# yaramohamadi/Pairwise_Sample_Optimization

Hardware: AMD Instinct MI355X
Metric: PSO train-step imgs/sec (paired 1024² SDXL) at 1/2/4/8 MI355X (higher is better)
Workload: dtype bf16; 1 GPU; C2: SDXL-Turbo PSO train step, LoRA r=32 grads, 2 pairs/GPU/micro-step, gas 2, 2-step sampler (T=1); global_batch=4, seq_len=4096, resolution=1024, parallelism=dp1, launch=eager

## Files before the change

### include/pso_amd.h

```cpp
#ifndef PSO_AMD_H
#define PSO_AMD_H

#include <stddef.h>
#include <stdint.h>

#ifdef __cplusplus
extern "C" {
#endif

#define PSO_ABI_VERSION 1

#define PSO_OK 0
#define PSO_ERR_ARG 1
#define PSO_ERR_HIP 2
#define PSO_ERR_UNSUPPORTED 3

#define PSO_F32 0
#define PSO_BF16 1
#define PSO_F16 2
#define PSO_U8 2

#define PSO_MODE_TURBO 0
#define PSO_MODE_DMD 1
#define PSO_MODE_DMD_F16 2
// ... 85 lines not shown
                    float grad_scale, void* deps, int deps_dtype, const void* ws, size_t ws_bytes, void* stream);

#define PSO_CONV_NORMAL 1
#define PSO_CONV_UP2 2
#define PSO_CONV_T2 3
int pso_conv2d(int mode, int B, const void* src1, int C1, const void* src2, int C2, int H, int W, int Ho, int Wo,
               int ks, int stride, int pad, const void* weight, int Cout, const void* a2, long lda2, int K2,
               const void* b2, long ldb2, float alpha, const void* bias, const void* rowbias, long ld_rowbias,
               const void* resid, long ldr, void* out, long ldo, int out_dtype, int accumulate, void* stream);
size_t pso_conv2d_ws_bytes(int B, int Ho, int Wo, int Cout, int K1, int K2);
int pso_conv2d_ws(int mode, int B, const void* src1, int C1, const void* src2, int C2, int H, int W, int Ho, int Wo,
                  int ks, int stride, int pad, const void* weight, int Cout, const void* a2, long lda2, int K2,
                  const void* b2, long ldb2, float alpha, const void* bias, const void* rowbias, long ld_rowbias,
                  const void* resid, long ldr, void* out, long ldo, int out_dtype, int accumulate, void* ws,
                  size_t ws_bytes, void* stream);

size_t pso_group_norm_ws_bytes(int B, int HW, int C);
int pso_group_norm_fwd(int B, int HW, int C, int G, float eps, const void* x, const void* gamma, const void* beta,
                       int silu, void* y, float* stats, void* ws, size_t ws_bytes, void* stream);
int pso_group_norm_bwd(int B, int HW, int C, int G, const void* x, const void* dy, const float* stats,
                       const void* gamma, const void* beta, int silu, const void* dadd, void* dx, float* dgamma,
                       float* dbeta, int accumulate_dparams, void* ws, size_t ws_bytes, void* stream);

int pso_layer_norm_fwd(int M, int C, float eps, const void* x, long ldx, const void* gamma, const void* beta, void* y,
                       long ldy, float* stats, void* stream);
int pso_layer_norm_bwd(int M, int C, const void* x, long ldx, const void* dy, long lddy, const float* stats,
                       const void* gamma, const void* dadd, long ldadd, void* dx, long lddx, void* stream);

int pso_attention_fwd(int B, int H, int Sq, int Sk, const void* q, long ldq, long sq_b, const void* k, long ldk,
                      long sk_b, const void* v, long ldv, long sv_b, float scale, void* o, long ldo, long so_b,
// ... 124 lines not shown
```

### pairwise_sample_optimization_amd/_lib.py

```python
import ctypes
import os

import torch

_HERE = os.path.dirname(os.path.abspath(__file__))
KNOBS = os.environ.get("PSO_LIB", "") == "knobs"
F16 = os.environ.get("PSO_LIB", "") == "f16"
LIB_PATH = os.environ.get("PSO_LIB_PATH") or os.path.join(
    _HERE, "libpso_amd_knobs.so" if KNOBS else "libpso_amd_f16.so" if F16 else "libpso_amd.so")

PSO_F32 = 0
PSO_BF16 = 1
PSO_F16 = 2
ELEM_DTYPE = torch.float16 if F16 else torch.bfloat16
ELEM_CODE = PSO_F16 if F16 else PSO_BF16
MODE_TURBO = 0
MODE_DMD = 1
MODE_DMD_F16 = 2
MODE_DMD_BF16 = 3
COEF_STRIDE = 8
AMP_WORDS = 16
(AMP_SCALE, AMP_INV_SCALE, AMP_FOUND_INF, AMP_GROWTH_TRACKER, AMP_STEP, AMP_SKIPPED, AMP_NORM, AMP_CLIP_COEF,
 AMP_GRAD_MUL, AMP_BC1, AMP_BC2_SQRT, AMP_C1, AMP_C2) = range(13)
AMP_INT_WORDS = (AMP_FOUND_INF, AMP_GROWTH_TRACKER, AMP_STEP, AMP_SKIPPED)
# ... 49 lines not shown
    "pso_gemm_tn_ws": (ci, [ci, ci, ci, vp, cl, vp, cl, cf, vp, cl, vp, csz, vp]),
    "pso_gemm_tn_rank_batch": (ci, [ci, ci, ci, vp, vp]),
    "pso_gemm_tn_rank_batch_ws_bytes": (csz, [ci, ci, ci, vp]),
    "pso_gemm_tn_rank_batch_ws": (ci, [ci, ci, ci, vp, vp, csz, vp]),
    "pso_gemm_skinny_grouped": (ci, [ci, ci, ci, vp, cl, vp, cl, cf, vp, cl, ci, vp]),
    "pso_gemm_geglu": (ci, [ci, ci, vp, cl, ci, vp, cl, vp, vp, cl, vp, cl, ci, vp]),
    "pso_gemm_geglu_bwd": (ci, [ci, ci, vp, cl, ci, vp, cl, vp, cl, vp, cl, vp]),
    "pso_quant_rows_fp8": (ci, [ci, ci, vp, cl, vp, cl, vp, vp]),
    "pso_gemm_fp8": (ci, [ci, ci, ci, ci, vp, cl, vp, vp, cl, vp, vp, cl, ci, vp, vp, cl, vp, ci, ci, cf, vp, vp, cl,
                          vp, cl, vp, cl, ci, vp]),
    "pso_conv2d": (ci, [ci, ci, vp, ci, vp, ci, ci, ci, ci, ci, ci, ci, ci, vp, ci, vp, cl, ci, vp, cl, cf, vp, vp,
                        cl, vp, cl, vp, cl, ci, ci, vp]),
    "pso_conv2d_ws_bytes": (csz, [ci, ci, ci, ci, ci, ci]),
    "pso_conv2d_ws": (ci, [ci, ci, vp, ci, vp, ci, ci, ci, ci, ci, ci, ci, ci, vp, ci, vp, cl, ci, vp, cl, cf, vp, vp,
                           cl, vp, cl, vp, cl, ci, ci, vp, csz, vp]),
    "pso_group_norm_ws_bytes": (csz, [ci, ci, ci]),
    "pso_group_norm_fwd": (ci, [ci, ci, ci, ci, cf, vp, vp, vp, ci, vp, vp, vp, csz, vp]),
    "pso_group_norm_bwd": (ci, [ci, ci, ci, ci, vp, vp, vp, vp, vp, ci, vp, vp, vp, vp, ci, vp, csz, vp]),
    "pso_layer_norm_fwd": (ci, [ci, ci, cf, vp, cl, vp, vp, vp, cl, vp, vp]),
    "pso_layer_norm_bwd": (ci, [ci, ci, vp, cl, vp, cl, vp, vp, vp, cl, vp, cl, vp]),
    "pso_attention_fwd": (ci, [ci, ci, ci, ci, vp, cl, cl, vp, cl, cl, vp, cl, cl, cf, vp, cl, cl, vp, vp]),
    "pso_attention_bwd_ws_bytes": (csz, [ci, ci, ci, ci]),
    "pso_attention_bwd": (ci, [ci, ci, ci, ci, vp, cl, cl, vp, cl, cl, vp, cl, cl, vp, cl, cl, vp, vp, cl, cl, cf,
                               vp, cl, cl, vp, cl, cl, vp, cl, cl, vp, csz, vp]),
    "pso_geglu_fwd": (ci, [cl, ci, vp, cl, vp, cl, vp]),
    "pso_geglu_bwd": (ci, [cl, ci, vp, cl, vp, cl, vp, cl, vp]),
    "pso_silu": (ci, [cl, vp, vp, vp]),
    "pso_timestep_embedding": (ci, [ci, ci, vp, vp, cl, ci, vp]),
    "pso_transpose": (ci, [ci, ci, ci, vp, cl, vp, cl, vp]),
    "pso_im2col3": (ci, [ci, ci, ci, ci, vp, vp, ci, vp]),
# ... 129 lines not shown
```

### pairwise_sample_optimization_amd/csrc/elementwise.hip

```cpp
#include "common.h"

__device__ __forceinline__ void unpack8e(uint4 v, float* f) {
  const uint32_t w[4] = {v.x, v.y, v.z, v.w};
#pragma unroll
  for (int i = 0; i < 4; ++i) {
    f[2 * i] = bf2f(w[i] & 0xffff);
    f[2 * i + 1] = bf2f(w[i] >> 16);
  }
}
__device__ __forceinline__ uint4 pack8e(const float* f) {
  return make_uint4(pack2bf(f[0], f[1]), pack2bf(f[2], f[3]), pack2bf(f[4], f[5]), pack2bf(f[6], f[7]));
}

static int grid_for(long n, int per_thread = 1) {
  long g = (n / per_thread + 255) / 256;
  if (g > 8192) g = 8192;
  return (int)(g < 1 ? 1 : g);
}

#define GRID_STRIDE(i, n) for (long i = blockIdx.x * (long)blockDim.x + threadIdx.x; i < (n); i += (long)gridDim.x * blockDim.x)


__global__ void geglu_fwd_kernel(long M, int F, const bf16_t* __restrict__ in, long ldi, bf16_t* __restrict__ out,
                                 long ldo) {
// ... 209 lines not shown
    const bf16_t* src = w + co * ldw + (long)tap * Ci + ci;
    if (vec && co < Co && ci + 8 <= Ci) {
      *reinterpret_cast<uint4*>(&tile[r][c]) = *reinterpret_cast<const uint4*>(src);
    } else {
      for (int e = 0; e < 8; ++e) tile[r][c + e] = (co < Co && ci + e < Ci) ? src[e] : (bf16_t)0;
    }
  }
  __syncthreads();
  const int lx = t & 63, ly = t >> 6;
  for (int i = ly; i < 64; i += 4) {
    const int ci = ci0 + i, co = co0 + lx;
    if (ci < Ci && co < Co) wt[((long)ci * ks * ks + tap2) * Co + co] = tile[lx][i];
  }
}

__global__ void concat_kernel(long npix, int C1, const bf16_t* __restrict__ x1, int C2, const bf16_t* __restrict__ x2,
                              bf16_t* __restrict__ out) {
  const int C8 = (C1 + C2) / 8, c18 = C1 / 8;
  GRID_STRIDE(v, npix * C8) {
    const long p = v / C8;
    const int ch = (int)(v - p * C8);
    const uint4 val = ch < c18 ? *reinterpret_cast<const uint4*>(x1 + p * C1 + ch * 8)
                               : *reinterpret_cast<const uint4*>(x2 + p * C2 + (ch - c18) * 8);
    *reinterpret_cast<uint4*>(out + v * 8) = val;
  }
}

__global__ void split_kernel(long npix, int C1, int C2, const bf16_t* __restrict__ in, bf16_t* __restrict__ y1,
                             bf16_t* __restrict__ y2, const bf16_t* __restrict__ add2) {
  const int C8 = (C1 + C2) / 8, c18 = C1 / 8;
// ... 236 lines not shown
  cast_f32_bf16_kernel<<<grid_for(n, 8), 256, 0, (hipStream_t)stream>>>(n, x, scale, (bf16_t*)y);
  return pso_check_launch("pso_cast_f32_bf16");
}

int pso_cast_bf16_f32(long n, const void* x, float* y, void* stream) {
  cast_bf16_f32_kernel<<<grid_for(n, 8), 256, 0, (hipStream_t)stream>>>(n, (const bf16_t*)x, y);
  return pso_check_launch("pso_cast_bf16_f32");
}

int pso_conv_weight_t(int Co, int ks, int Ci, int flip, const void* w, void* wt, void* stream) {
  conv_weight_t_kernel<<<dim3(cdiv(Ci, 64), cdiv(Co, 64), ks * ks), 256, 0, (hipStream_t)stream>>>(
      Co, ks, Ci, flip, (const bf16_t*)w, (bf16_t*)wt);
  return pso_check_launch("pso_conv_weight_t");
}

}
```

### pairwise_sample_optimization_amd/csrc/gemm.hip

```cpp
#include "common.h"

#include <cstdlib>

#define GEMM_THREADS 256
#define BK 64

struct ConvGeom {
  int mode;
  const bf16_t* src2;
  int C1, C2;
  int H, W;
  int Ho, Wo;
  int ks, stride, pad;
};

struct GemmArgs {
  const bf16_t* a1; long lda1; int K1;
  const bf16_t* b1; long ldb1;
  const bf16_t* a2; long lda2; int K2;
  const bf16_t* b2; long ldb2;
  int tail_group_n;
  int tail_m;
  int M, N;
  ConvGeom conv;
// ... 151 lines not shown
  const int nt2 = (g.a2 && m0 < g.tail_m) ? (g.K2 + BK - 1) / BK : 0;
  const int nt_all = nt1 + nt2;
  const int per = (nt_all + gridDim.y - 1) / gridDim.y;
  const int t_beg = blockIdx.y * per;
  const int t_end = min(nt_all, t_beg + per);
  const int nt = t_end > t_beg ? t_end - t_beg : 0;
  const long a2_off = g.tail_group_n > 0 ? (long)(n0 / g.tail_group_n) * g.K2 : 0;

  const int prow = lane >> 3;
  const int pch = lane & 7;
  const bf16_t* zero = reinterpret_cast<const bf16_t*>(g_zero16);
  const long zb = blockIdx.z;
  const bf16_t* const a1 = g.a1 + zb * g.bat_a;
  const bf16_t* const b1 = g.b1 + zb * g.bat_b;
  void* const outp = reinterpret_cast<char*>(g.out) + zb * g.bat_o * (g.out_dtype == PSO_F32 ? 4 : 2);
  const int K1 = g.K1;
  int lcA[T::A_CH], offA[T::A_CH];
  int lcB[T::B_CH], offB[T::B_CH];
  RowCoord rc[T::A_CH];
#pragma unroll
  for (int i = 0; i < T::A_CH; ++i) {
    const int R = pa(i) * 8 + prow;
    const int m = min(m0 + R, g.M - 1);
    lcA[i] = pch ^ (R & 7);
    offA[i] = CONV ? 0 : (int)((long)m * g.lda1) + lcA[i] * 8;
    if (CONV) {
      const int hw = g.conv.Ho * g.conv.Wo;
      rc[i].valid = true;
      rc[i].b = m / hw;
      const int rem = m - rc[i].b * hw;
// ... 21 lines not shown
        const TapInfo ti = tap_info(g, k0);
#pragma unroll
        for (int i = 0; i < T::A_CH; ++i) {
          const int piece = pa(i);
          int iy, ix;
          bool ok;
          if (CONV == PSO_CONV_NORMAL) {
            iy = rc[i].oy * cvS + ti.kh - cvP;
            ix = rc[i].ox * cvS + ti.kw - cvP;
            ok = (unsigned)iy < (unsigned)cvH && (unsigned)ix < (unsigned)cvW;
          } else if (CONV == PSO_CONV_UP2) {
            const int uy = rc[i].oy + ti.kh - cvP, ux = rc[i].ox + ti.kw - cvP;
            ok = (unsigned)uy < (unsigned)(2 * cvH) && (unsigned)ux < (unsigned)(2 * cvW);
            iy = uy >> 1;
            ix = ux >> 1;
          } else {
            const int ty = rc[i].oy + cvP - ti.kh, tx = rc[i].ox + cvP - ti.kw;
            iy = ty >> 1;
            ix = tx >> 1;
            ok = ty >= 0 && tx >= 0 && !(ty & 1) && !(tx & 1) && iy < cvH && ix < cvW;
          }
          const bf16_t* src = ti.src + ((long)((rc[i].b * cvH + iy) * cvW + ix)) * ti.Cs + ti.c0 + lcA[i] * 8;
          __builtin_amdgcn_global_load_lds(static_cast<const void*>(ok ? src : zero), (lds_void*)(la + piece * 8 * BK), 16, 0, 0);
        }
      } else {
#pragma unroll
        for (int i = 0; i < T::A_CH; ++i) {
          const int piece = pa(i);
          const bool ok = full || k0 + lcA[i] * 8 < K1;
          __builtin_amdgcn_global_load_lds(static_cast<const void*>(ok ? a1 + offA[i] + k0 : zero), (lds_void*)(la + piece * 8 * BK), 16, 0, 0);
// ... 308 lines not shown
#pragma unroll
      for (int it = 0; it < ITERS; ++it) {
        const int q = threadIdx.x + it * NT;
        const int ml = q / CC, cl = (q - (q / CC) * CC) * 8;
        const int m = m0 + ml;
        if (q >= BM * CC || m >= g.M) continue;
        uint4 y = *reinterpret_cast<const uint4*>(tl + ml * TP + cl);
        if (g.resid) {
          const uint32_t yw[4] = {y.x, y.y, y.z, y.w}, rw[4] = {rr[it].x, rr[it].y, rr[it].z, rr[it].w};
          uint32_t o[4];
#pragma unroll
          for (int e = 0; e < 4; ++e)
            o[e] = pack2bf(bf2f(yw[e] & 0xffff) + bf2f(rw[e] & 0xffff), bf2f(yw[e] >> 16) + bf2f(rw[e] >> 16));
          y = make_uint4(o[0], o[1], o[2], o[3]);
        }
        *reinterpret_cast<uint4*>(reinterpret_cast<bf16_t*>(outp) + (long)m * g.ldo + n0 + cl) = y;
      }
      return;
    }
  }
  if (!PIPE && epi_fast && nt > 0) {
    epi_prefetch();
    const bool has_add = g.resid || g.rowbias;
#pragma unroll
    for (int i = 0; i < MI; ++i) {
      const int m = m0 + wm * (BM / WM) + i * 16 + fr;
      if (m >= g.M) continue;
#pragma unroll
      for (int j = 0; j < NJ; ++j) {
        const int n = n0 + wn * (BN / WN) + j * 16 + fk * 4;
        float v[4] = {acc[i][j][0] * g.alpha + bf2f(ebias[j].x & 0xffff), acc[i][j][1] * g.alpha + bf2f(ebias[j].x >> 16),
                      acc[i][j][2] * g.alpha + bf2f(ebias[j].y & 0xffff), acc[i][j][3] * g.alpha + bf2f(ebias[j].y >> 16)};
        if (has_add) {
          v[0] += bf2f(eadd[i][j].x & 0xffff); v[1] += bf2f(eadd[i][j].x >> 16);
          v[2] += bf2f(eadd[i][j].y & 0xffff); v[3] += bf2f(eadd[i][j].y >> 16);
        }
        if (g.out_dtype == PSO_ELEM) {
          *reinterpret_cast<uint2*>(reinterpret_cast<bf16_t*>(outp) + (long)m * g.ldo + n) =
              make_uint2(pack2bf(v[0], v[1]), pack2bf(v[2], v[3]));
        } else {
          float4* o = reinterpret_cast<float4*>(reinterpret_cast<float*>(outp) + (long)m * g.ldo + n);
          if (g.accumulate) {
            const float4 old = *o;
            v[0] += old.x; v[1] += old.y; v[2] += old.z; v[3] += old.w;
          }
          *o = make_float4(v[0], v[1], v[2], v[3]);
        }
      }
    }
    return;
  }
#pragma unroll
  for (int i = 0; i < MI; ++i) {
    const int m = m0 + wm * (BM / WM) + i * 16 + fr;
    if (m >= g.M) continue;
#pragma unroll
    for (int j = 0; j < NJ; ++j) {
      const int n = n0 + wn * (BN / WN) + j * 16 + fk * 4;
      if (n >= g.N) continue;
      float v[4] = {acc[i][j][0] * g.alpha, acc[i][j][1] * g.alpha, acc[i][j][2] * g.alpha,
                    acc[i][j][3] * g.alpha};
      if (gridDim.y > 1) {
        float* o = reinterpret_cast<float*>(outp) + (long)m * g.ldo + n;
        for (int r = 0; r < 4 && n + r < g.N; ++r) atomicAdd(o + r, v[r]);
        continue;
      }
      const bool full = g.vec_ok && (n + 4 <= g.N);
      if (full) {
        if (g.bias) {
          const uint2 bv = *reinterpret_cast<const uint2*>(g.bias + n);
          v[0] += bf2f(bv.x & 0xffff); v[1] += bf2f(bv.x >> 16); v[2] += bf2f(bv.y & 0xffff); v[3] += bf2f(bv.y >> 16);
        }
        if (g.rowbias) {
          const uint2 bv = *reinterpret_cast<const uint2*>(g.rowbias + (long)(m / g.rows_per_group) * g.ld_rowbias + n);
          v[0] += bf2f(bv.x & 0xffff); v[1] += bf2f(bv.x >> 16); v[2] += bf2f(bv.y & 0xffff); v[3] += bf2f(bv.y >> 16);
        }
        if (g.resid) {
          const uint2 rv = *reinterpret_cast<const uint2*>(g.resid + (long)m * g.ldr + n);
          v[0] += bf2f(rv.x & 0xffff); v[1] += bf2f(rv.x >> 16); v[2] += bf2f(rv.y & 0xffff); v[3] += bf2f(rv.y >> 16);
        }
        if (g.out_dtype == PSO_ELEM) {
          *reinterpret_cast<uint2*>(reinterpret_cast<bf16_t*>(outp) + (long)m * g.ldo + n) =
              make_uint2(pack2bf(v[0], v[1]), pack2bf(v[2], v[3]));
        } else {
          float4* o = reinterpret_cast<float4*>(reinterpret_cast<float*>(outp) + (long)m * g.ldo + n);
          if (g.accumulate) {
            const float4 old = *o;
            v[0] += old.x; v[1] += old.y; v[2] += old.z; v[3] += old.w;
          }
          *o = make_float4(v[0], v[1], v[2], v[3]);
        }
      } else {
        for (int r = 0; r < 4 && n + r < g.N; ++r) {
          float x = v[r];
          if (g.bias) x += bf2f(g.bias[n + r]);
          if (g.rowbias) x += bf2f(g.rowbias[(long)(m / g.rows_per_group) * g.ld_rowbias + n + r]);
          if (g.resid) x += bf2f(g.resid[(long)m * g.ldr + n + r]);
          if (g.out_dtype == PSO_ELEM) {
            reinterpret_cast<bf16_t*>(outp)[(long)m * g.ldo + n + r] = f2bf(x);
          } else {
            float* o = reinterpret_cast<float*>(outp) + (long)m * g.ldo + n + r;
            *o = g.accumulate ? *o + x : x;
          }
        }
      }
    }
  }
}

template <int BM, int BN, int WM = 2, int WN = 2, int STAGES = 2, bool PIPE = false, int EPI = EPI_NONE>
static int launch(const GemmArgs& g, hipStream_t st, int ksplit = 1) {
  const int nblk = ((g.M + BM - 1) / BM) * ((g.N + BN - 1) / BN);
  dim3 grid(nblk, ksplit, g.batch > 1 ? g.batch : 1);
  const int threads = 64 * WM * WN;
  const size_t shm = (size_t)STAGES * (BM + BN) * BK * sizeof(bf16_t);
  pso_note_kernel("gemm_bf16_kernel<%d, %d, %d, %d, %d, %d, %s, %d>", BM, BN, EPI != EPI_NONE ? 0 : g.conv.mode, WM, WN,
                  STAGES, PIPE ? "true" : "false", EPI);
  static bool attr_done = false;
  if constexpr (EPI != EPI_NONE) {
    if (!attr_done) {
      (void)hipFuncSetAttribute((const void*)gemm_bf16_kernel<BM, BN, 0, WM, WN, STAGES, PIPE, EPI>,
                                hipFuncAttributeMaxDynamicSharedMemorySize, (int)shm);
      attr_done = true;
    }
    gemm_bf16_kernel<BM, BN, 0, WM, WN, STAGES, PIPE, EPI><<<grid, threads, shm, st>>>(g);
    return pso_check_launch("pso_gemm(geglu)");
  }
  if (!attr_done) {
    (void)hipFuncSetAttribute((const void*)gemm_bf16_kernel<BM, BN, 0, WM, WN, STAGES, PIPE, EPI>,
                        hipFuncAttributeMaxDynamicSharedMemorySize, (int)shm);
    (void)hipFuncSetAttribute((const void*)gemm_bf16_kernel<BM, BN, PSO_CONV_NORMAL, WM, WN, STAGES, PIPE, EPI>,
                        hipFuncAttributeMaxDynamicSharedMemorySize, (int)shm);
    (void)hipFuncSetAttribute((const void*)gemm_bf16_kernel<BM, BN, PSO_CONV_UP2, WM, WN, STAGES, PIPE, EPI>,
                        hipFuncAttributeMaxDynamicSharedMemorySize, (int)shm);
    (void)hipFuncSetAttribute((const void*)gemm_bf16_kernel<BM, BN, PSO_CONV_T2, WM, WN, STAGES, PIPE, EPI>,
                        hipFuncAttributeMaxDynamicSharedMemorySize, (int)shm);
    attr_done = true;
  }
  switch (g.conv.mode) {
    case PSO_CONV_NORMAL:
      gemm_bf16_kernel<BM, BN, PSO_CONV_NORMAL, WM, WN, STAGES, PIPE, EPI><<<grid, threads, shm, st>>>(g);
      break;
    case PSO_CONV_UP2: gemm_bf16_kernel<BM, BN, PSO_CONV_UP2, WM, WN, STAGES, PIPE, EPI><<<grid, threads, shm, st>>>(g); break;
    case PSO_CONV_T2: gemm_bf16_kernel<BM, BN, PSO_CONV_T2, WM, WN, STAGES, PIPE, EPI><<<grid, threads, shm, st>>>(g); break;
    default: gemm_bf16_kernel<BM, BN, 0, WM, WN, STAGES, PIPE, EPI><<<grid, threads, shm, st>>>(g);
  }
  return pso_check_launch("pso_gemm");
}

static bool al16(const void* p) { return ((uintptr_t)p & 15) == 0; }
static bool al8(const void* p) { return ((uintptr_t)p & 7) == 0; }

// ... 102 lines not shown
  g.group_m = g_gemm_group > 0 ? g_gemm_group : PSO_GEMM_GROUP_M;
  if (g.tail_group_n > 0 && (g.tail_group_n % 64) != 0) {
    pso_set_error("pso_gemm: tail_group_n must be a multiple of 64");
    return PSO_ERR_ARG;
  }
  g.stage_epi = gv_raw != 41 && g.out_dtype == PSO_ELEM && al16(g.out) && (g.ldo % 8) == 0 &&
                (!g.resid || (al16(g.resid) && (g.ldr % 8) == 0));
  g.vec_ok = (g.ldo % 4) == 0 && (g.out_dtype == PSO_F32 ? al16(g.out) : al8(g.out)) &&
             (!g.resid || ((g.ldr % 4) == 0 && al8(g.resid))) && (!g.bias || al8(g.bias)) &&
             (!g.rowbias || (al8(g.rowbias) && (g.ld_rowbias % 4) == 0));
  const bool bn64_only = g.tail_group_n > 0 && (g.tail_group_n % 128) != 0;
  const bool bn256_ok = g.tail_group_n == 0 || (g.tail_group_n % 256) == 0;
  const long Ktot = (long)g.K1 + (g.a2 ? g.K2 : 0);
  if (g.batch > 1) {
    auto tl = [&](int bm, int bn) { return (long)((g.M + bm - 1) / bm) * ((g.N + bn - 1) / bn) * g.batch; };
    if ((g.N % 160) == 0 && tl(128, 160) >= 256) return launch<128, 160, 2, 2, 2>(g, st);
    if (tl(128, 128) >= 256) return launch<128, 128, 2, 4, 2>(g, st);
    return launch<64, 64>(g, st);
  }
  if (g.ws) {
    const SplitPlan sp = gemm_split_plan(g.M, g.N, g.K1, g.K2, g.a2 != nullptr, true);
    if (sp.ks >= 2) {
      if (sp.bn == 160) launch<128, 160, 2, 2, 2>(g, st, sp.ks);
      else launch<128, 128, 2, 4, 2>(g, st, sp.ks);
      const long n4 = (long)g.M * (g.N / 4);
      gemm_splitk_reduce_kernel<<<(unsigned)((n4 + 255) / 256), 256, 0, st>>>(g, sp.ks);
      return pso_check_launch("pso_gemm_ws");
    }
    g.ws = nullptr;
  }
// ... 678 lines not shown
  g.alpha = alpha; g.rows_per_group = 1;
  g.out = out; g.ldo = ldo; g.out_dtype = out_dtype;
  g.bat_a = stride_a; g.bat_b = stride_b; g.bat_o = stride_o; g.batch = batch;
  return run_gemm(g, (hipStream_t)stream);
}

int pso_conv2d(int mode, int B, const void* src1, int C1, const void* src2, int C2, int H, int W, int Ho, int Wo,
               int ks, int stride, int pad, const void* weight, int Cout, const void* a2, long lda2, int K2,
               const void* b2, long ldb2, float alpha, const void* bias, const void* rowbias, long ld_rowbias,
               const void* resid, long ldr, void* out, long ldo, int out_dtype, int accumulate, void* stream) {
  PSO_ARG_CHECK(mode == PSO_CONV_NORMAL || mode == PSO_CONV_UP2 || mode == PSO_CONV_T2, "pso_conv2d: bad mode");
  PSO_ARG_CHECK(src1 && weight && out, "pso_conv2d: null operand");
  PSO_ARG_CHECK((C1 % 64) == 0 && (C2 % 64) == 0 && (C2 == 0 || src2),
                "pso_conv2d: channel sources must be multiples of 64 (C1=%d C2=%d); use im2col for small C", C1, C2);
  PSO_ARG_CHECK(al16(src1) && (!src2 || al16(src2)) && al16(weight), "pso_conv2d: alignment");
  PSO_ARG_CHECK(ks == 1 || ks == 3, "pso_conv2d: ks must be 1 or 3");
  PSO_ARG_CHECK(mode != PSO_CONV_UP2 || (Ho == 2 * H && Wo == 2 * W && stride == 1), "pso_conv2d: UP2 geometry");
  PSO_ARG_CHECK(!a2 || ((K2 % 8) == 0 && b2 && al16(a2) && al16(b2)), "pso_conv2d: bad second operand");
  PSO_DTYPE_CHECK(out_dtype, "pso_conv2d");
  PSO_ARG_CHECK(!accumulate || out_dtype == PSO_F32, "pso_conv2d: accumulate needs f32 output");
  if (mode == PSO_CONV_NORMAL && ks == 3 && stride == 1 && pad == 1 && Ho == H && Wo == W && C2 == 0 && !a2 &&
      !rowbias && !resid && alpha == 1.f && out_dtype == PSO_ELEM && !accumulate && ldo == Cout && Cout <= 3 &&
      pso_conv3x3_smallc_run(B, H, W, C1, Cout, src1, weight, bias, out, (hipStream_t)stream) == PSO_OK)
    return PSO_OK;
  GemmArgs g{};
  const int Ct = C1 + C2;
  g.a1 = (const bf16_t*)src1; g.lda1 = 0; g.K1 = ks * ks * Ct;
  g.b1 = (const bf16_t*)weight; g.ldb1 = g.K1;
  g.a2 = (const bf16_t*)a2; g.lda2 = lda2; g.K2 = a2 ? K2 : 0;
  g.b2 = (const bf16_t*)b2; g.ldb2 = ldb2;
  g.M = B * Ho * Wo; g.N = Cout;
// ... 13 lines not shown
  if (M <= 0 || M > 0x7fffffffL) return 0;
  const SplitPlan sp = gemm_split_plan((int)M, Cout, K1, K2, K2 > 0, true);
  return sp.ks >= 2 ? (size_t)sp.ks * M * Cout * sizeof(float) : 0;
}

int pso_conv2d_ws(int mode, int B, const void* src1, int C1, const void* src2, int C2, int H, int W, int Ho, int Wo,
                  int ks, int stride, int pad, const void* weight, int Cout, const void* a2, long lda2, int K2,
                  const void* b2, long ldb2, float alpha, const void* bias, const void* rowbias, long ld_rowbias,
                  const void* resid, long ldr, void* out, long ldo, int out_dtype, int accumulate, void* ws,
                  size_t ws_bytes, void* stream) {
  PSO_ARG_CHECK(mode == PSO_CONV_NORMAL || mode == PSO_CONV_UP2 || mode == PSO_CONV_T2, "pso_conv2d_ws: bad mode");
  PSO_ARG_CHECK(src1 && weight && out, "pso_conv2d_ws: null operand");
  PSO_ARG_CHECK((C1 % 64) == 0 && (C2 % 64) == 0 && (C2 == 0 || src2),
                "pso_conv2d_ws: channel sources must be multiples of 64 (C1=%d C2=%d)", C1, C2);
  PSO_ARG_CHECK(al16(src1) && (!src2 || al16(src2)) && al16(weight), "pso_conv2d_ws: alignment");
  PSO_ARG_CHECK(ks == 1 || ks == 3, "pso_conv2d_ws: ks must be 1 or 3");
  PSO_ARG_CHECK(mode != PSO_CONV_UP2 || (Ho == 2 * H && Wo == 2 * W && stride == 1), "pso_conv2d_ws: UP2 geometry");
  PSO_ARG_CHECK(!a2 || ((K2 % 8) == 0 && b2 && al16(a2) && al16(b2)), "pso_conv2d_ws: bad second operand");
  PSO_DTYPE_CHECK(out_dtype, "pso_conv2d_ws");
  PSO_ARG_CHECK(!accumulate || out_dtype == PSO_F32, "pso_conv2d_ws: accumulate needs f32 output");
  GemmArgs g{};
  const int Ct = C1 + C2;
  g.a1 = (const bf16_t*)src1; g.lda1 = 0; g.K1 = ks * ks * Ct;
  g.b1 = (const bf16_t*)weight; g.ldb1 = g.K1;
  g.a2 = (const bf16_t*)a2; g.lda2 = lda2; g.K2 = a2 ? K2 : 0;
  g.b2 = (const bf16_t*)b2; g.ldb2 = ldb2;
  g.M = B * Ho * Wo; g.N = Cout;
  g.tail_m = g.M;
  g.conv.mode = mode; g.conv.src2 = (const bf16_t*)src2; g.conv.C1 = C1; g.conv.C2 = C2;
  g.conv.H = H; g.conv.W = W; g.conv.Ho = Ho; g.conv.Wo = Wo; g.conv.ks = ks; g.conv.stride = stride; g.conv.pad = pad;
  g.alpha = alpha;
  g.bias = (const bf16_t*)bias;
  g.rowbias = (const bf16_t*)rowbias; g.ld_rowbias = ld_rowbias; g.rows_per_group = Ho * Wo;
  g.resid = (const bf16_t*)resid; g.ldr = ldr;
  g.out = out; g.ldo = ldo; g.out_dtype = out_dtype; g.accumulate = accumulate;
  const SplitPlan sp = gemm_split_plan(g.M, g.N, g.K1, g.K2, g.a2 != nullptr, true);
  const bool ok = ws && (((uintptr_t)ws) & 15) == 0 && sp.ks >= 2 && ws_bytes >= (size_t)sp.ks * g.M * g.N * sizeof(float) &&
                  (ldo % 4) == 0 && (out_dtype == PSO_F32 ? al16(out) : al8(out)) && (g.N % 4) == 0 &&
                  (!resid || ((ldr % 4) == 0 && al8(resid))) && (!rowbias || (ld_rowbias % 4) == 0) &&
                  gemm_ws_allowed();
  g.ws = ok ? (float*)ws : nullptr;
  return run_gemm(g, (hipStream_t)stream);
}

int pso_gemm_geglu(int M, int N, const void* a, long lda, int K, const void* w, long ldw, const void* bias, void* out,
                   long ldo, void* out_pre, long ld_pre, int pre_rows, void* stream) {
  PSO_ARG_CHECK(M > 0 && N > 0 && (N % 256) == 0 && K > 0 && (K % 8) == 0 && a && w && bias && out,
                "pso_gemm_geglu: need N %% 256 == 0, K %% 8 == 0, bias");
  PSO_ARG_CHECK(al16(a) && al16(w) && (lda % 8) == 0 && (ldw % 8) == 0 && al16(out) && (ldo % 8) == 0 && al8(bias) &&
                    (!out_pre || (al16(out_pre) && (ld_pre % 8) == 0)),
                "pso_gemm_geglu: alignment (16-B rows)");
  PSO_ARG_CHECK((long)M * lda < 0x7fffffffL && (long)N * ldw < 0x7fffffffL, "pso_gemm_geglu: operand too large");
  GemmArgs g{};
  g.a1 = (const bf16_t*)a; g.lda1 = lda; g.K1 = K;
  g.b1 = (const bf16_t*)w; g.ldb1 = ldw;
  g.M = M; g.N = N; g.alpha = 1.f;
// ... 152 lines not shown
```

### pairwise_sample_optimization_amd/kernels.py

```python
import ctypes
import os

import torch

from . import _lib
from ._lib import check, lib, ptr, require_cuda, stream_ptr, dtype_code, PSO_BF16, PSO_F32

CONV_NORMAL, CONV_UP2, CONV_T2 = 1, 2, 3
ELEM = _lib.ELEM_DTYPE

PROFILE = None


def _prof_begin():
    if PROFILE is None:
        return None
    e0 = torch.cuda.Event(enable_timing=True)
    e0.record()
    return e0


def _prof_end(e0, flops, nbytes=0.0, tag=None):
    if e0 is not None:
        e1 = torch.cuda.Event(enable_timing=True)
# ... 701 lines not shown

def cast_bf16_f32(x, out=None):
    out = torch.empty(x.shape, device=x.device, dtype=torch.float32) if out is None else out
    check(lib().pso_cast_bf16_f32(x.numel(), ptr(x.contiguous()), ptr(out), stream_ptr()), "pso_cast_bf16_f32")
    return out


def conv_weight_t(w, flip):
    Co, ks, _, Ci = w.shape
    out = torch.empty((Ci, ks, ks, Co), device=w.device, dtype=w.dtype)
    check(lib().pso_conv_weight_t(Co, ks, Ci, int(flip), ptr(w.contiguous()), ptr(out), stream_ptr()),
          "pso_conv_weight_t")
    return out


def concat_channels(x1, x2):
    C1, C2 = x1.shape[-1], x2.shape[-1]
    out = torch.empty(x1.shape[:-1] + (C1 + C2,), device=x1.device, dtype=x1.dtype)
    npix = x1.numel() // C1
    check(lib().pso_concat_channels(npix, C1, ptr(x1.contiguous()), C2, ptr(x2.contiguous()), ptr(out),
                                    stream_ptr()), "pso_concat_channels")
    return out


def split_channels(x, C1, add2=None):
    C = x.shape[-1]
    C2 = C - C1
    y1 = torch.empty(x.shape[:-1] + (C1,), device=x.device, dtype=x.dtype)
    y2 = torch.empty(x.shape[:-1] + (C2,), device=x.device, dtype=x.dtype)
    npix = x.numel() // C
# ... 412 lines not shown
```

### pairwise_sample_optimization_amd/unet.py

```python
import math
import os
from dataclasses import dataclass, field, replace
from types import SimpleNamespace

import torch
import torch.nn as nn

from . import _lib
from . import kernels as K

ELEM = _lib.ELEM_DTYPE
TN_BATCH = os.environ.get("PSO_TN_BATCH", "1") != "0"


@dataclass
class UNetConfig:
    in_channels: int = 4
    out_channels: int = 4
    block_out_channels: tuple = (320, 640, 1280)
    layers_per_block: int = 2
    transformer_layers_per_block: tuple = (1, 2, 10)
    down_has_attn: tuple = (False, True, True)
    head_dim: int = 64
    cross_attention_dim: int = 2048
# ... 871 lines not shown

    def fwd(self, x, rt):
        if rt.save:
            rt.saved.append({"hw": x.shape[1:3], "x": x if rt.fg is not None else None})
        return K.conv2d(x, self.conv.w_nhwc, stride=2, bias=self.conv.bias)

    def bwd(self, dy, rt):
        sv = rt.saved.pop()
        if rt.fg is not None:
            _conv_dw(rt.fg, self.conv, dy.reshape(-1, self.conv.cout), sv["x"], rt,
                     lambda x: K.im2col_conv(x, stride=2))
        return K.conv2d(dy, self.conv.w_dx, mode=K.CONV_T2, out_hw=tuple(sv["hw"]))


class Upsample2D(nn.Module):
    def __init__(self, C):
        super().__init__()
        self.conv = Conv2d(C, C, 3)

    def prepare(self):
        self.conv.prepare()

    def fwd(self, x, rt):
        if rt.save and rt.fg is not None:
            rt.saved.append({"x": x})
        return K.conv2d(x, self.conv.w_nhwc, mode=K.CONV_UP2, bias=self.conv.bias)

    def bwd(self, dy, rt):
        if rt.fg is not None:
            _conv_dw(rt.fg, self.conv, dy.reshape(-1, self.conv.cout), rt.saved.pop()["x"], rt,
                     lambda x: K.im2col_conv(x, mode=K.CONV_UP2))
        du = K.conv2d(dy, self.conv.w_dx)
        return K.sumpool2(du)


class _Block(nn.Module):

    def __init__(self):
        super().__init__()


class TimestepEmbedding(nn.Module):
    def __init__(self, fin, dim):
        super().__init__()
        self.linear_1 = Linear(fin, dim)
        self.linear_2 = Linear(dim, dim)
# ... 564 lines not shown
```

### pairwise_sample_optimization_amd/vae.py

```python
import math
from dataclasses import dataclass
from types import SimpleNamespace

import torch
import torch.nn as nn

from . import _lib
from . import kernels as K
from .unet import Conv2d, Linear, Norm, ResnetBlock2D, Upsample2D

ELEM = _lib.ELEM_DTYPE


@dataclass
class VAEConfig:
    latent_channels: int = 4
    out_channels: int = 3
    block_out_channels: tuple = (128, 256, 512, 512)
    layers_per_block: int = 2
    norm_num_groups: int = 32
    scaling_factor: float = 0.13025

    @staticmethod
    def tiny():
# ... 35 lines not shown
        super().__init__()
        ch = list(reversed(cfg.block_out_channels))
        G = cfg.norm_num_groups
        self.conv_in = Conv2d(cfg.latent_channels, ch[0], 3)
        mid = _Blk()
        mid.resnets = nn.ModuleList([ResnetBlock2D(ch[0], ch[0], G, 1e-6, 0), ResnetBlock2D(ch[0], ch[0], G, 1e-6, 0)])
        mid.attentions = nn.ModuleList([VAEAttention(ch[0], G)])
        self.mid_block = mid
        self.up_blocks = nn.ModuleList()
        prev = ch[0]
        for i, c in enumerate(ch):
            blk = _Blk()
            blk.resnets = nn.ModuleList([ResnetBlock2D(prev if j == 0 else c, c, G, 1e-6, 0)
                                         for j in range(cfg.layers_per_block + 1)])
            if i < len(ch) - 1:
                blk.upsamplers = nn.ModuleList([Upsample2D(c)])
            prev = c
            self.up_blocks.append(blk)
        self.conv_norm_out = Norm(ch[-1])
        self.conv_out = Conv2d(ch[-1], cfg.out_channels, 3)


class Downsample2DEnc(nn.Module):

    def __init__(self, C):
        super().__init__()
        self.conv = Conv2d(C, C, 3, stride=2)

    def prepare(self):
        self.conv.prepare()

# ... 193 lines not shown
```

Measured before the change: 38.06 imgs/s.

## Fold nearest-upsample into 2x2 phase convolutions for VAE decoder upsamplers

Adds a sub-pixel (phase) decomposition of the nearest-2x upsample followed by 3x3 conv. The 3x3 weights are pre-folded into four 2x2 phase kernels, so the forward GEMM runs over the low-resolution input with K=4C instead of 9C on the upsampled grid. It also adds a folded 4x4 stride-2 backward-data kernel that replaces the conv plus sumpool2. This removes redundant MACs and the separate pooling pass in the VAE decoder upsamplers. The cost is extra folded weight storage and a new scatter-style output row mapping in the GEMM epilogue.

```diff
diff --git a/include/pso_amd.h b/include/pso_amd.h
--- a/include/pso_amd.h
+++ b/include/pso_amd.h
@@ -123,6 +123,11 @@
                   const void* b2, long ldb2, float alpha, const void* bias, const void* rowbias, long ld_rowbias,
                   const void* resid, long ldr, void* out, long ldo, int out_dtype, int accumulate, void* ws,
                   size_t ws_bytes, void* stream);
+#define PSO_CONV_UP2P 4
+int pso_conv2d_up2p(int B, const void* src, int C, int H, int W, const void* weight, int Cout, const void* bias,
+                    void* out, long ldo, int out_dtype, void* stream);
+int pso_conv_fold_up2(int Cout, int C, const void* w, void* out, void* stream);
+int pso_conv_fold_dx4(int Cin, int Cout, const void* wdx, void* out, void* stream);
 
 size_t pso_group_norm_ws_bytes(int B, int HW, int C);
 int pso_group_norm_fwd(int B, int HW, int C, int G, float eps, const void* x, const void* gamma, const void* beta,
diff --git a/pairwise_sample_optimization_amd/_lib.py b/pairwise_sample_optimization_amd/_lib.py
--- a/pairwise_sample_optimization_amd/_lib.py
+++ b/pairwise_sample_optimization_amd/_lib.py
@@ -87,6 +87,9 @@
     "pso_conv2d_ws_bytes": (csz, [ci, ci, ci, ci, ci, ci]),
     "pso_conv2d_ws": (ci, [ci, ci, vp, ci, vp, ci, ci, ci, ci, ci, ci, ci, ci, vp, ci, vp, cl, ci, vp, cl, cf, vp, vp,
                            cl, vp, cl, vp, cl, ci, ci, vp, csz, vp]),
+    "pso_conv2d_up2p": (ci, [ci, vp, ci, ci, ci, vp, ci, vp, vp, cl, ci, vp]),
+    "pso_conv_fold_up2": (ci, [ci, ci, vp, vp, vp]),
+    "pso_conv_fold_dx4": (ci, [ci, ci, vp, vp, vp]),
     "pso_group_norm_ws_bytes": (csz, [ci, ci, ci]),
     "pso_group_norm_fwd": (ci, [ci, ci, ci, ci, cf, vp, vp, vp, ci, vp, vp, vp, csz, vp]),
     "pso_group_norm_bwd": (ci, [ci, ci, ci, ci, vp, vp, vp, vp, vp, ci, vp, vp, vp, vp, ci, vp, csz, vp]),
diff --git a/pairwise_sample_optimization_amd/csrc/elementwise.hip b/pairwise_sample_optimization_amd/csrc/elementwise.hip
--- a/pairwise_sample_optimization_amd/csrc/elementwise.hip
+++ b/pairwise_sample_optimization_amd/csrc/elementwise.hip
@@ -247,6 +247,32 @@
   }
 }
 
+template <bool FWD>
+__global__ void conv_fold_kernel(int R, int C, const bf16_t* __restrict__ in, bf16_t* __restrict__ out) {
+  constexpr int T = FWD ? 2 : 4, P = FWD ? 4 : 1;
+  const int C8 = C / 8;
+  GRID_STRIDE(v, (long)P * R * T * T * C8) {
+    const int c = (int)(v % C8) * 8;
+    long q = v / C8;
+    const int b = (int)(q % T); q /= T;
+    const int a = (int)(q % T); q /= T;
+    const int r = (int)(q % R);
+    const int p = (int)(q / R);
+    const int py = p >> 1, px = p & 1;
+    const int rlo = FWD ? (a ? 1 + py : 0) : max(a - 1, 0), rhi = FWD ? (a ? 2 : py) : min(a, 2);
+    const int clo = FWD ? (b ? 1 + px : 0) : max(b - 1, 0), chi = FWD ? (b ? 2 : px) : min(b, 2);
+    float acc[8] = {0, 0, 0, 0, 0, 0, 0, 0};
+    for (int kh = rlo; kh <= rhi; ++kh)
+      for (int kw = clo; kw <= chi; ++kw) {
+        float w[8];
+        unpack8e(*reinterpret_cast<const uint4*>(in + ((long)r * 9 + kh * 3 + kw) * C + c), w);
+#pragma unroll
+        for (int j = 0; j < 8; ++j) acc[j] += w[j];
+      }
+    *reinterpret_cast<uint4*>(out + v * 8) = pack8e(acc);
+  }
+}
+
 __global__ void concat_kernel(long npix, int C1, const bf16_t* __restrict__ x1, int C2, const bf16_t* __restrict__ x2,
                               bf16_t* __restrict__ out) {
   const int C8 = (C1 + C2) / 8, c18 = C1 / 8;
@@ -513,4 +539,21 @@
   return pso_check_launch("pso_conv_weight_t");
 }
 
-}
+int pso_conv_fold_up2(int Cout, int C, const void* w, void* out, void* stream) {
+  PSO_ARG_CHECK(Cout > 0 && C > 0 && (C % 8) == 0 && w && out && ((uintptr_t)w & 15) == 0 && ((uintptr_t)out & 15) == 0,
+                "pso_conv_fold_up2: need C %% 8 == 0 and 16-B aligned weights");
+  conv_fold_kernel<true><<<grid_for(16L * Cout * (C / 8)), 256, 0, (hipStream_t)stream>>>(Cout, C, (const bf16_t*)w,
+                                                                                           (bf16_t*)out);
+  return pso_check_launch("pso_conv_fold_up2");
+}
+
+int pso_conv_fold_dx4(int Cin, int Cout, const void* wdx, void* out, void* stream) {
+  PSO_ARG_CHECK(Cin > 0 && Cout > 0 && (Cout % 8) == 0 && wdx && out && ((uintptr_t)wdx & 15) == 0 &&
+                    ((uintptr_t)out & 15) == 0,
+                "pso_conv_fold_dx4: need Cout %% 8 == 0 and 16-B aligned weights");
+  conv_fold_kernel<false><<<grid_for(16L * Cin * (Cout / 8)), 256, 0, (hipStream_t)stream>>>(Cin, Cout, (const bf16_t*)wdx,
+                                                                                             (bf16_t*)out);
+  return pso_check_launch("pso_conv_fold_dx4");
+}
+
+}
diff --git a/pairwise_sample_optimization_amd/csrc/gemm.hip b/pairwise_sample_optimization_amd/csrc/gemm.hip
--- a/pairwise_sample_optimization_amd/csrc/gemm.hip
+++ b/pairwise_sample_optimization_amd/csrc/gemm.hip
@@ -189,6 +189,14 @@
   const bf16_t* const a1 = g.a1 + zb * g.bat_a;
   const bf16_t* const b1 = g.b1 + zb * g.bat_b;
   void* const outp = reinterpret_cast<char*>(g.out) + zb * g.bat_o * (g.out_dtype == PSO_F32 ? 4 : 2);
+  const int ppy = CONV == PSO_CONV_UP2P ? (int)(blockIdx.z >> 1) : 0, ppx = CONV == PSO_CONV_UP2P ? (int)(blockIdx.z & 1) : 0;
+  auto orow = [&](int m) -> long {
+    if (CONV != PSO_CONV_UP2P) return m;
+    const int hw = g.conv.Ho * g.conv.Wo;
+    const int b = m / hw, rem = m - b * hw;
+    const int oy = rem / g.conv.Wo, ox = rem - oy * g.conv.Wo;
+    return ((long)(b * 2 * g.conv.Ho + 2 * oy + ppy)) * (2 * g.conv.Wo) + 2 * ox + ppx;
+  };
   const int K1 = g.K1;
   int lcA[T::A_CH], offA[T::A_CH];
   int lcB[T::B_CH], offB[T::B_CH];
@@ -240,6 +248,10 @@
             ok = (unsigned)uy < (unsigned)(2 * cvH) && (unsigned)ux < (unsigned)(2 * cvW);
             iy = uy >> 1;
             ix = ux >> 1;
+          } else if (CONV == PSO_CONV_UP2P) {
+            iy = rc[i].oy + ti.kh - 1 + ppy;
+            ix = rc[i].ox + ti.kw - 1 + ppx;
+            ok = (unsigned)iy < (unsigned)cvH && (unsigned)ix < (unsigned)cvW;
           } else {
             const int ty = rc[i].oy + cvP - ti.kh, tx = rc[i].ox + cvP - ti.kw;
             iy = ty >> 1;
@@ -578,7 +590,7 @@
             o[e] = pack2bf(bf2f(yw[e] & 0xffff) + bf2f(rw[e] & 0xffff), bf2f(yw[e] >> 16) + bf2f(rw[e] >> 16));
           y = make_uint4(o[0], o[1], o[2], o[3]);
         }
-        *reinterpret_cast<uint4*>(reinterpret_cast<bf16_t*>(outp) + (long)m * g.ldo + n0 + cl) = y;
+        *reinterpret_cast<uint4*>(reinterpret_cast<bf16_t*>(outp) + orow(m) * g.ldo + n0 + cl) = y;
       }
       return;
     }
@@ -590,6 +602,7 @@
     for (int i = 0; i < MI; ++i) {
       const int m = m0 + wm * (BM / WM) + i * 16 + fr;
       if (m >= g.M) continue;
+      const long mo = orow(m);
 #pragma unroll
       for (int j = 0; j < NJ; ++j) {
         const int n = n0 + wn * (BN / WN) + j * 16 + fk * 4;
@@ -600,10 +613,10 @@
           v[2] += bf2f(eadd[i][j].y & 0xffff); v[3] += bf2f(eadd[i][j].y >> 16);
         }
         if (g.out_dtype == PSO_ELEM) {
-          *reinterpret_cast<uint2*>(reinterpret_cast<bf16_t*>(outp) + (long)m * g.ldo + n) =
+          *reinterpret_cast<uint2*>(reinterpret_cast<bf16_t*>(outp) + mo * g.ldo + n) =
               make_uint2(pack2bf(v[0], v[1]), pack2bf(v[2], v[3]));
         } else {
-          float4* o = reinterpret_cast<float4*>(reinterpret_cast<float*>(outp) + (long)m * g.ldo + n);
+          float4* o = reinterpret_cast<float4*>(reinterpret_cast<float*>(outp) + mo * g.ldo + n);
           if (g.accumulate) {
             const float4 old = *o;
             v[0] += old.x; v[1] += old.y; v[2] += old.z; v[3] += old.w;
@@ -618,6 +631,7 @@
   for (int i = 0; i < MI; ++i) {
     const int m = m0 + wm * (BM / WM) + i * 16 + fr;
     if (m >= g.M) continue;
+    const long mo = orow(m);
 #pragma unroll
     for (int j = 0; j < NJ; ++j) {
       const int n = n0 + wn * (BN / WN) + j * 16 + fk * 4;
@@ -625,7 +639,7 @@
       float v[4] = {acc[i][j][0] * g.alpha, acc[i][j][1] * g.alpha, acc[i][j][2] * g.alpha,
                     acc[i][j][3] * g.alpha};
       if (gridDim.y > 1) {
-        float* o = reinterpret_cast<float*>(outp) + (long)m * g.ldo + n;
+        float* o = reinterpret_cast<float*>(outp) + mo * g.ldo + n;
         for (int r = 0; r < 4 && n + r < g.N; ++r) atomicAdd(o + r, v[r]);
         continue;
       }
@@ -644,10 +658,10 @@
           v[0] += bf2f(rv.x & 0xffff); v[1] += bf2f(rv.x >> 16); v[2] += bf2f(rv.y & 0xffff); v[3] += bf2f(rv.y >> 16);
         }
         if (g.out_dtype == PSO_ELEM) {
-          *reinterpret_cast<uint2*>(reinterpret_cast<bf16_t*>(outp) + (long)m * g.ldo + n) =
+          *reinterpret_cast<uint2*>(reinterpret_cast<bf16_t*>(outp) + mo * g.ldo + n) =
               make_uint2(pack2bf(v[0], v[1]), pack2bf(v[2], v[3]));
         } else {
-          float4* o = reinterpret_cast<float4*>(reinterpret_cast<float*>(outp) + (long)m * g.ldo + n);
+          float4* o = reinterpret_cast<float4*>(reinterpret_cast<float*>(outp) + mo * g.ldo + n);
           if (g.accumulate) {
             const float4 old = *o;
             v[0] += old.x; v[1] += old.y; v[2] += old.z; v[3] += old.w;
@@ -661,9 +675,9 @@
           if (g.rowbias) x += bf2f(g.rowbias[(long)(m / g.rows_per_group) * g.ld_rowbias + n + r]);
           if (g.resid) x += bf2f(g.resid[(long)m * g.ldr + n + r]);
           if (g.out_dtype == PSO_ELEM) {
-            reinterpret_cast<bf16_t*>(outp)[(long)m * g.ldo + n + r] = f2bf(x);
+            reinterpret_cast<bf16_t*>(outp)[mo * g.ldo + n + r] = f2bf(x);
           } else {
-            float* o = reinterpret_cast<float*>(outp) + (long)m * g.ldo + n + r;
+            float* o = reinterpret_cast<float*>(outp) + mo * g.ldo + n + r;
             *o = g.accumulate ? *o + x : x;
           }
         }
@@ -681,6 +695,9 @@
   pso_note_kernel("gemm_bf16_kernel<%d, %d, %d, %d, %d, %d, %s, %d>", BM, BN, EPI != EPI_NONE ? 0 : g.conv.mode, WM, WN,
                   STAGES, PIPE ? "true" : "false", EPI);
   static bool attr_done = false;
+  constexpr bool UP2P_TILE = EPI == EPI_NONE && !PIPE && STAGES == 2 &&
+                             ((BM == 256 && BN == 256 && WM == 2 && WN == 4) || (BM == 128 && BN == 160 && WM == 2 && WN == 2) ||
+                              (BM == 128 && BN == 128 && WM == 2 && WN == 4) || (BM == 64 && BN == 64 && WM == 2 && WN == 2));
   if constexpr (EPI != EPI_NONE) {
     if (!attr_done) {
       (void)hipFuncSetAttribute((const void*)gemm_bf16_kernel<BM, BN, 0, WM, WN, STAGES, PIPE, EPI>,
@@ -699,7 +716,19 @@
                         hipFuncAttributeMaxDynamicSharedMemorySize, (int)shm);
     (void)hipFuncSetAttribute((const void*)gemm_bf16_kernel<BM, BN, PSO_CONV_T2, WM, WN, STAGES, PIPE, EPI>,
                         hipFuncAttributeMaxDynamicSharedMemorySize, (int)shm);
+    if constexpr (UP2P_TILE)
+      (void)hipFuncSetAttribute((const void*)gemm_bf16_kernel<BM, BN, PSO_CONV_UP2P, WM, WN, STAGES, PIPE, EPI>,
+                                hipFuncAttributeMaxDynamicSharedMemorySize, (int)shm);
     attr_done = true;
+  }
+  if (g.conv.mode == PSO_CONV_UP2P) {
+    if constexpr (UP2P_TILE) {
+      gemm_bf16_kernel<BM, BN, PSO_CONV_UP2P, WM, WN, STAGES, PIPE, EPI><<<grid, threads, shm, st>>>(g);
+      return pso_check_launch("pso_conv2d_up2p");
+    } else {
+      pso_set_error("pso_conv2d_up2p: no %d x %d phase-conv tile", BM, BN);
+      return PSO_ERR_ARG;
+    }
   }
   switch (g.conv.mode) {
     case PSO_CONV_NORMAL:
@@ -832,6 +861,7 @@
   const long Ktot = (long)g.K1 + (g.a2 ? g.K2 : 0);
   if (g.batch > 1) {
     auto tl = [&](int bm, int bn) { return (long)((g.M + bm - 1) / bm) * ((g.N + bn - 1) / bn) * g.batch; };
+    if (g.conv.mode == PSO_CONV_UP2P && (g.N % 256) == 0 && tl(256, 256) >= 1024) return launch<256, 256, 2, 4, 2>(g, st);
     if ((g.N % 160) == 0 && tl(128, 160) >= 256) return launch<128, 160, 2, 2, 2>(g, st);
     if (tl(128, 128) >= 256) return launch<128, 128, 2, 4, 2>(g, st);
     return launch<64, 64>(g, st);
@@ -1540,7 +1570,8 @@
   PSO_ARG_CHECK((C1 % 64) == 0 && (C2 % 64) == 0 && (C2 == 0 || src2),
                 "pso_conv2d: channel sources must be multiples of 64 (C1=%d C2=%d); use im2col for small C", C1, C2);
   PSO_ARG_CHECK(al16(src1) && (!src2 || al16(src2)) && al16(weight), "pso_conv2d: alignment");
-  PSO_ARG_CHECK(ks == 1 || ks == 3, "pso_conv2d: ks must be 1 or 3");
+  PSO_ARG_CHECK(ks == 1 || ks == 3 || (mode == PSO_CONV_NORMAL && (ks == 2 || ks == 4)),
+                "pso_conv2d: ks must be 1 or 3 (2 or 4 also in PSO_CONV_NORMAL)");
   PSO_ARG_CHECK(mode != PSO_CONV_UP2 || (Ho == 2 * H && Wo == 2 * W && stride == 1), "pso_conv2d: UP2 geometry");
   PSO_ARG_CHECK(!a2 || ((K2 % 8) == 0 && b2 && al16(a2) && al16(b2)), "pso_conv2d: bad second operand");
   PSO_DTYPE_CHECK(out_dtype, "pso_conv2d");
@@ -1584,7 +1615,8 @@
   PSO_ARG_CHECK((C1 % 64) == 0 && (C2 % 64) == 0 && (C2 == 0 || src2),
                 "pso_conv2d_ws: channel sources must be multiples of 64 (C1=%d C2=%d)", C1, C2);
   PSO_ARG_CHECK(al16(src1) && (!src2 || al16(src2)) && al16(weight), "pso_conv2d_ws: alignment");
-  PSO_ARG_CHECK(ks == 1 || ks == 3, "pso_conv2d_ws: ks must be 1 or 3");
+  PSO_ARG_CHECK(ks == 1 || ks == 3 || (mode == PSO_CONV_NORMAL && (ks == 2 || ks == 4)),
+                "pso_conv2d_ws: ks must be 1 or 3 (2 or 4 also in PSO_CONV_NORMAL)");
   PSO_ARG_CHECK(mode != PSO_CONV_UP2 || (Ho == 2 * H && Wo == 2 * W && stride == 1), "pso_conv2d_ws: UP2 geometry");
   PSO_ARG_CHECK(!a2 || ((K2 % 8) == 0 && b2 && al16(a2) && al16(b2)), "pso_conv2d_ws: bad second operand");
   PSO_DTYPE_CHECK(out_dtype, "pso_conv2d_ws");
@@ -1610,6 +1642,31 @@
                   (!resid || ((ldr % 4) == 0 && al8(resid))) && (!rowbias || (ld_rowbias % 4) == 0) &&
                   gemm_ws_allowed();
   g.ws = ok ? (float*)ws : nullptr;
+  return run_gemm(g, (hipStream_t)stream);
+}
+
+int pso_conv2d_up2p(int B, const void* src, int C, int H, int W, const void* weight, int Cout, const void* bias,
+                    void* out, long ldo, int out_dtype, void* stream) {
+  PSO_ARG_CHECK(src && weight && out, "pso_conv2d_up2p: null operand");
+  PSO_ARG_CHECK(B > 0 && H > 0 && W > 0 && Cout > 0 && C > 0 && (C % 64) == 0,
+                "pso_conv2d_up2p: need positive sizes and C %% 64 == 0 (C=%d)", C);
+  PSO_ARG_CHECK(al16(src) && al16(weight), "pso_conv2d_up2p: alignment");
+  PSO_DTYPE_CHECK(out_dtype, "pso_conv2d_up2p");
+  PSO_ARG_CHECK(4L * B * H * W < 0x7fffffffL && (long)B * H * W * C < (1L << 40) && 4L * Cout * C < 0x7fffffffL &&
+                    ldo >= Cout,
+                "pso_conv2d_up2p: geometry too large (or ldo < Cout)");
+  GemmArgs g{};
+  g.a1 = (const bf16_t*)src; g.lda1 = 0; g.K1 = 4 * C;
+  g.b1 = (const bf16_t*)weight; g.ldb1 = g.K1;
+  g.M = B * H * W; g.N = Cout;
+  g.tail_m = g.M;
+  g.conv.mode = PSO_CONV_UP2P; g.conv.C1 = C;
+  g.conv.H = H; g.conv.W = W; g.conv.Ho = H; g.conv.Wo = W; g.conv.ks = 2; g.conv.stride = 1; g.conv.pad = 1;
+  g.alpha = 1.f;
+  g.bias = (const bf16_t*)bias;
+  g.rows_per_group = 1;
+  g.out = out; g.ldo = ldo; g.out_dtype = out_dtype;
+  g.batch = 4; g.bat_a = 0; g.bat_b = (long)Cout * g.K1; g.bat_o = 0;
   return run_gemm(g, (hipStream_t)stream);
 }
 
diff --git a/pairwise_sample_optimization_amd/kernels.py b/pairwise_sample_optimization_amd/kernels.py
--- a/pairwise_sample_optimization_amd/kernels.py
+++ b/pairwise_sample_optimization_amd/kernels.py
@@ -739,6 +739,41 @@
     return out
 
 
+def conv_fold_up2(w):
+    require_cuda(w)
+    Co, ks, ks2, Ci = w.shape
+    assert ks == 3 and ks2 == 3 and w.is_contiguous() and w.dtype == ELEM
+    out = torch.empty((4, Co, 2, 2, Ci), device=w.device, dtype=w.dtype)
+    check(lib().pso_conv_fold_up2(Co, Ci, ptr(w), ptr(out), stream_ptr()), "pso_conv_fold_up2")
+    return out
+
+
+def conv_fold_dx4(w_dx):
+    require_cuda(w_dx)
+    Ci, ks, ks2, Co = w_dx.shape
+    assert ks == 3 and ks2 == 3 and w_dx.is_contiguous() and w_dx.dtype == ELEM
+    out = torch.empty((Ci, 4, 4, Co), device=w_dx.device, dtype=w_dx.dtype)
+    check(lib().pso_conv_fold_dx4(Ci, Co, ptr(w_dx), ptr(out), stream_ptr()), "pso_conv_fold_dx4")
+    return out
+
+
+def conv2d_up2(x, w_up2p, *, bias=None, out=None, out_dtype=ELEM):
+    require_cuda(x, w_up2p)
+    B, H, W, C = x.shape
+    P, Cout, k1, k2, Ci = w_up2p.shape
+    assert (P, k1, k2, Ci) == (4, 2, 2, C) and x.is_contiguous() and w_up2p.is_contiguous()
+    if out is None:
+        out = torch.empty((B, 2 * H, 2 * W, Cout), device=x.device, dtype=out_dtype)
+    assert out.shape == (B, 2 * H, 2 * W, Cout) and out.is_contiguous()
+    e0 = _prof_begin()
+    check(lib().pso_conv2d_up2p(B, ptr(x), C, H, W, ptr(w_up2p), Cout, ptr(bias), ptr(out), Cout, dtype_code(out),
+                                stream_ptr()), "pso_conv2d_up2p")
+    _prof_end(e0, 2.0 * B * H * W * Cout * 16 * C,
+              2.0 * (B * H * W * C + 16 * Cout * C) + out.element_size() * 4 * B * H * W * Cout,
+              ("conv", 4, B, H, W, C, 0, Cout, 2, 1, 0))
+    return out
+
+
 def concat_channels(x1, x2):
     C1, C2 = x1.shape[-1], x2.shape[-1]
     out = torch.empty(x1.shape[:-1] + (C1 + C2,), device=x1.device, dtype=x1.dtype)
diff --git a/pairwise_sample_optimization_amd/unet.py b/pairwise_sample_optimization_amd/unet.py
--- a/pairwise_sample_optimization_amd/unet.py
+++ b/pairwise_sample_optimization_amd/unet.py
@@ -909,22 +909,31 @@
 
 
 class Upsample2D(nn.Module):
-    def __init__(self, C):
+
+    def __init__(self, C, fold=False):
         super().__init__()
         self.conv = Conv2d(C, C, 3)
+        self.fold = fold
 
     def prepare(self):
         self.conv.prepare()
+        if self.fold:
+            self.w_up2p = K.conv_fold_up2(self.conv.w_nhwc)
+            self.w_dx4 = K.conv_fold_dx4(self.conv.w_dx)
 
     def fwd(self, x, rt):
         if rt.save and rt.fg is not None:
             rt.saved.append({"x": x})
+        if self.fold:
+            return K.conv2d_up2(x, self.w_up2p, bias=self.conv.bias)
         return K.conv2d(x, self.conv.w_nhwc, mode=K.CONV_UP2, bias=self.conv.bias)
 
     def bwd(self, dy, rt):
         if rt.fg is not None:
             _conv_dw(rt.fg, self.conv, dy.reshape(-1, self.conv.cout), rt.saved.pop()["x"], rt,
                      lambda x: K.im2col_conv(x, mode=K.CONV_UP2))
+        if self.fold:
+            return K.conv2d(dy, self.w_dx4, stride=2, pad=1)
         du = K.conv2d(dy, self.conv.w_dx)
         return K.sumpool2(du)
 
diff --git a/pairwise_sample_optimization_amd/vae.py b/pairwise_sample_optimization_amd/vae.py
--- a/pairwise_sample_optimization_amd/vae.py
+++ b/pairwise_sample_optimization_amd/vae.py
@@ -73,7 +73,7 @@
             blk.resnets = nn.ModuleList([ResnetBlock2D(prev if j == 0 else c, c, G, 1e-6, 0)
                                          for j in range(cfg.layers_per_block + 1)])
             if i < len(ch) - 1:
-                blk.upsamplers = nn.ModuleList([Upsample2D(c)])
+                blk.upsamplers = nn.ModuleList([Upsample2D(c, fold=True)])
             prev = c
             self.up_blocks.append(blk)
         self.conv_norm_out = Norm(ch[-1])
```

Result: no change. 38.03 imgs/s (-0.1%).
